# iscc/iscc-search

Hardware: AMD Instinct MI355X
Metric: queries/sec (+ roofline of the dominant kernel), 64-bit Hamming k=10 over 100M codes, exact top-k (higher is better)
Workload: dtype fp4 (e2m1 0/1 x +-1 products, f32 accumulation: exact integers)

## Files before the change

iscc_search_amd/csrc/isccsearch.hip:

```cpp
#include <hip/hip_runtime.h>

#include <algorithm>
#include <cerrno>
#include <cstdarg>
#include <cstdio>
#include <cmath>
#include <condition_variable>
#include <cstring>
#include <memory>
#include <mutex>
#include <string>
#include <unordered_map>
#include <thread>
#include <atomic>
#include <functional>
#include <chrono>
#include <vector>

#include "../../include/isccsearch.h"
#include "kernels.hip.h"
#include "mfma_scan.h"
#include "docfreq.h"
#include "simprint_score.h"
#include "asset_score.h"
// ... 110 lines not shown
        hipError_t e = hipHostMalloc((void**)&p, want * sizeof(T), hipHostMallocDefault);
        if (e != hipSuccess) { p = nullptr; (void)hipGetLastError(); return fail(-ENOMEM, "hipHostMalloc(%zu bytes) failed: %s", want * sizeof(T), hipGetErrorString(e)); }
        n = want;
        return 0;
    }
    void release() { if (p) (void)hipHostFree(p); p = nullptr; n = 0; }
};

constexpr size_t DIRECT_RESULT_BYTES = 1 << 20;

uint64_t mask_for(uint32_t pbytes) {
    const uint32_t rem = pbytes & 7;
    return rem ? ~0ULL << (8 * (8 - rem)) : ~0ULL;
}
uint32_t next_pow2(uint32_t v) { uint32_t p = 2; while (p < v) p <<= 1; return p; }

}

struct PendingSearch;
struct isccsearch_handle {
    std::mutex mu;
    std::mutex qmu;
    std::condition_variable qcv;
    std::vector<PendingSearch*> pending;
    bool leader_active = false;
    int device = 0;
    int cus = 256;
    hipStream_t stream = nullptr;
    std::vector<std::unique_ptr<Table>> tables;
    int tq = 8;
    bool profile = false;
    bool count_candidates = false;
    bool nontemporal = true;
    uint32_t blocks_per_cu = 8;
    uint64_t boot_rows = 65536;
    uint64_t level_growth = 8;
    bool repick = true;
    uint32_t tiny_rows = 16384;
    uint32_t select_wide_from = 2048;
    uint32_t fold_tau = 11;
    uint64_t stretch_bytes = CACHE_STRETCH_BYTES;
    uint64_t mfma_stretch_factor = 3;
    bool mfma = true;
    uint32_t mfma_pack_min_queries = 9;
    uint64_t mfma_few_rows = 12ull << 20;
    uint32_t mfma_min_queries = 17;
    uint32_t self_boot_per_k = 1024;
    bool spec_suppress = false;
    int device_search_hint = -1;
    int self_hint = 1;
    int speculate = 1;
    uint32_t spec_max_queries = 128;
    int mfma_pack = 1;
    uint64_t mfma_min_rows = 65536;
    bool self_tighten = true;
    bool boot_multi = true;
    uint32_t candidate_cap = 16384;
    uint32_t self_refresh_steps = 1;
    uint32_t self_max_k = ISCCSEARCH_MAX_K;
    uint64_t self_boot_rows = 65536;
    uint64_t mfma_level_growth = 4;
    uint16_t* d_rank = nullptr;
    DevBuf<uint64_t> d_queries;
    DevBuf<uint32_t> d_bias, d_cnt, d_ghist, d_overflow, d_listcnt, d_outcnt, d_freq;
    DevBuf<float> d_thr;
    DevBuf<uint64_t> d_cand;
    DevBuf<isk::Record> d_lists, d_final;
    PinBuf<uint64_t> p_queries;
    PinBuf<uint32_t> p_flags;
    DevBuf<unsigned char> d_block;
    PinBuf<unsigned char> p_block;
    DevBuf<uint64_t> d_misc;
    DevBuf<uint64_t> d_misc2;
    std::vector<isk::Record> h_final;
    std::vector<uint32_t> h_cnt, h_overflow;
    DevBuf<isk::Record> d_sp_rec;
    DevBuf<uint32_t> d_sp_rows, d_sp_nbest, d_sp_offs, d_sp_freqq, d_sp_unknown, d_sp_entry[2], d_sp_order[2], d_sp_matches, d_sp_nassets;
    DevBuf<uint32_t> d_sp_cnt, d_sp_dofg;
    DevBuf<unsigned char> d_sp_best, d_sp_temp;
    DevBuf<uint64_t> d_sp_asset[2];
    DevBuf<double> d_sp_score[2], d_sp_tab, d_sp_ws, d_sp_idfq;
    PinBuf<double> p_sp_tab;
    PinBuf<unsigned char> p_sp_out;
    uint32_t sp_tab_bits = 0, sp_tab_dup = 0xFFFFFFFFu;
    int64_t sp_tab_total = -1;
    DevBuf<isk::Record> d_am_rec, d_am_rec2;
    DevBuf<uint32_t> d_am_cnt, d_am_cnt2, d_am_off;
    DevBuf<iskas::Slot> d_am_slots;
    DevBuf<uint64_t> d_am_ex;
    DevBuf<uint8_t> d_am_hasex;
    DevBuf<double> d_am_tab;
    std::vector<double> am_tab;
    DevBuf<iskas::Item> d_am_scratch;
    PinBuf<unsigned char> p_am_out;
    size_t am_lds_allowed = 0;
    hipEvent_t ev_done = nullptr, ev_staged = nullptr, ev_producer = nullptr;
    bool ev_staged_pending = false;
    std::vector<std::pair<hipEvent_t, hipEvent_t>> ev_pool;
    std::vector<char> ev_level;
    size_t ev_used = 0;
    isccsearch_stats stats{};
};

namespace {

using H = isccsearch_handle;
// ... 232 lines not shown
        const Job& j = jobs[ji];
        Segment& s = *j.seg;
        Ctx c{};
        for (uint32_t w = 0; w < j.W; ++w) c.sp.col[w] = s.col[w];
        c.sp.queries = h->d_queries.p; c.sp.bias = h->d_bias.p; c.sp.cnt = h->d_cnt.p; c.sp.cand = h->d_cand.p;
        c.sp.ghist = h->d_ghist.p; c.sp.cap = cap; c.sp.k = k; c.sp.fold_tau = h->fold_tau; c.sp.nq_pad = nq_pad;
        c.sp.mask_lo = (uint32_t)j.mask_last; c.sp.mask_hi = (uint32_t)(j.mask_last >> 32);
        c.sp.thr_live = h->d_thr.p;
        c.sp.refresh_steps = h->self_refresh_steps;
        c.sl.cnt = h->d_cnt.p; c.sl.cand = h->d_cand.p; c.sl.cap = cap; c.sl.keys = s.keys;
        c.sl.rank = h->d_rank + (t.metric == ISCCSEARCH_METRIC_NPHD ? j.pbytes * 257 : 0);
        c.sl.out = multi ? h->d_lists.p + ji * (size_t)nq * k : d_out;
        c.sl.out_count = multi ? h->d_listcnt.p + ji * (size_t)nq : d_out_cnt;
        c.sl.overflow = d_flags + ji * (size_t)nq_pad;
        c.sl.k = k; c.sl.P = P; c.sl.prefix_bits = j.pbytes * 8; c.sl.q_base = 0;
        c.sl.overflow_count = mark_overflow ? isk::COUNT_OVERFLOW : 0;
        c.sl.out_rows = multi ? nullptr : d_out_rows;
        c.sl.out_kth = multi ? nullptr : d_out_kth;
        return c;
    }
    template <int NT>
    void launch_select_nt(const isk::SelectParams& sl, uint32_t blocks) const {
        if (sl.out_rows) {
            if (t.key_words == 2) hipLaunchKernelGGL((isk::select_kernel<2, true, NT>), dim3(blocks), dim3(NT), sel_lds, h->stream, sl);
            else hipLaunchKernelGGL((isk::select_kernel<1, true, NT>), dim3(blocks), dim3(NT), sel_lds, h->stream, sl);
        } else if (t.key_words == 2) hipLaunchKernelGGL((isk::select_kernel<2, false, NT>), dim3(blocks), dim3(NT), sel_lds, h->stream, sl);
        else hipLaunchKernelGGL((isk::select_kernel<1, false, NT>), dim3(blocks), dim3(NT), sel_lds, h->stream, sl);
    }
    void launch_select(const isk::SelectParams& sl, uint32_t blocks) const {
        const bool wide = sl.P >= h->select_wide_from && (sl.P >= 2 * h->select_wide_from || blocks <= (uint32_t)h->cus / 2);
        if (wide) launch_select_nt<1024>(sl, blocks);
        else launch_select_nt<isk::BLOCK>(sl, blocks);
    }
    bool tiny(const Job& j) const { return h->tiny_rows && j.seg->n <= h->tiny_rows && j.seg->n <= cap && j.seg->n < h->mfma_min_rows; }
    template <int NT>
    void launch_tiny_nt(const isk::TinyParams& tp, const isk::SelectParams& sl, const isk::InlineQueries& iq) const {
        if (sl.out_rows) {
            if (t.key_words == 2) hipLaunchKernelGGL((isk::tiny_search_kernel<2, true, NT>), dim3(nq), dim3(NT), sel_lds, h->stream, tp, sl, iq);
            else hipLaunchKernelGGL((isk::tiny_search_kernel<1, true, NT>), dim3(nq), dim3(NT), sel_lds, h->stream, tp, sl, iq);
        } else if (t.key_words == 2) hipLaunchKernelGGL((isk::tiny_search_kernel<2, false, NT>), dim3(nq), dim3(NT), sel_lds, h->stream, tp, sl, iq);
        else hipLaunchKernelGGL((isk::tiny_search_kernel<1, false, NT>), dim3(nq), dim3(NT), sel_lds, h->stream, tp, sl, iq);
    }
    size_t flag_words() const { return jobs.size() * (size_t)nq_pad; }

    bool use_mfma(const Job& j, uint64_t rows) const {
        const bool from_nine = j.pack || j.seg->n <= h->mfma_few_rows;
        return h->mfma && nq_pad >= (from_nine ? std::min(h->mfma_min_queries, h->mfma_pack_min_queries) : h->mfma_min_queries) && rows >= h->mfma_min_rows;
    }
    int scan(const Job& j, const isk::ScanParams& sp, int mode, bool sample) {
        const uint64_t rows = sp.n_rows - sp.row_begin;
        if (use_mfma(j, rows) || mode == isk::MODE_SELF) {
            const uint32_t g = isk::mfma_groups_per_chunk((int)j.W, nq_pad, j.pack);
            const uint32_t chunks = (nq_pad + g * 32 - 1) / (g * 32);
            const uint64_t rps = isk::mfma_rows_per_wave_step((int)j.W, j.pack);
            const uint64_t steps = (rows + rps - 1) / rps;
            const uint64_t wpb = isk::mfma_waves_per_block();
            const uint64_t bx = std::max<uint64_t>(1, std::min<uint64_t>((steps + wpb - 1) / wpb, std::max<uint32_t>(1, (uint32_t)h->cus * isk::mfma_blocks_per_cu((int)j.W, g, j.pack) / chunks)));
            const int e = isk::launch_mfma_scan((int)j.W, mode, j.pack, (uint32_t)bx, g, h->stream, sp);
            if (e) return fail(-EIO, "mfma scan: chunk of %u query groups does not fit the LDS budget (%s)", g, hipGetErrorString((hipError_t)e));
            h->stats.mfma_launches += 1;
            if (j.pack) h->stats.mfma_pack_launches += 1;
            h->stats.mfma_pair_words += rows * (uint64_t)nq * j.W;
            return 0;
        }
        if (mode != isk::MODE_COLLECT && mode != isk::MODE_STRETCH && mode != isk::MODE_BOTH) return fail(-EINVAL, "scan mode %d has no XOR + popcount kernel", mode);
        if (sp.n_rows / (uint64_t)tile_rows_for((int)j.W) >= (1ull << 31)) return fail(-E2BIG, "segment of %llu rows exceeds the scan kernel's 2^31 tiles", (unsigned long long)sp.n_rows);
        launch_scan((int)j.W, j.mask, tq, mode, h->nontemporal, dim3(scan_grid_x(h, j.W, rows, groups, sample), groups), h->stream, sp);
        return 0;
    }

    int begin(const uint64_t* hq) {
        jobs.clear();
        used_self = false;
        tq = h->tq;
        if (tq == 8 && nq > 8 && nq <= 16) tq = 16;
        nq_pad = (nq + tq - 1) / tq * tq;
        groups = nq_pad / tq;
        for (uint32_t b = 1; b <= ISCCSEARCH_MAX_BYTES; ++b) {
            Segment& s = t.seg[b];
            if (!s.n) continue;
            Job j;
            j.seg = &s;
            j.pbytes = t.metric == ISCCSEARCH_METRIC_NPHD ? std::min(b, qbytes) : b;
            j.W = (j.pbytes + 7) / 8;
            j.mask = (j.pbytes & 7) != 0;
            j.mask_last = mask_for(j.pbytes);
            j.pack = h->mfma_pack && j.W == 1;
            if (j.pack && j.pbytes == 8)
                for (uint32_t q = 0; q < nq && j.pack; ++q) j.pack = hq[(size_t)q * t.max_words] != 0;
            jobs.push_back(j);
        }
        if (jobs.empty()) {
            HIPOK(hipMemsetAsync(d_out_cnt, 0, nq * sizeof(uint32_t), h->stream));
            return 0;
        }
        cap = std::max<uint32_t>(h->candidate_cap, 16 * k);
        if (h->self_tighten && h->mfma && k <= h->self_max_k && radius < 0 && radius_ratio < 0) cap = std::max<uint32_t>(cap, 64 * k);
        multi = jobs.size() > 1;
        P = next_pow2(std::max<uint32_t>(std::max<uint32_t>(k, 1024), std::min<uint32_t>(4 * k, 4096)));
        sel_lds = (((size_t)P * 4 + 15) & ~(size_t)15) + (size_t)P * 8 * t.key_words + (d_out_rows ? (size_t)P * 4 : 0);
        int rc;
        if ((rc = h->d_queries.ensure((size_t)nq_pad * 4))) return rc;
        if ((rc = h->d_bias.ensure(nq_pad))) return rc;
        if ((rc = h->d_thr.ensure(nq_pad))) return rc;
        if ((rc = h->d_cnt.ensure((size_t)nq_pad * isk::CNT_STRIDE))) return rc;
        if ((rc = h->d_ghist.ensure((size_t)nq_pad * isk::HB))) return rc;
        if (!d_flags) {
            if ((rc = h->d_overflow.ensure(flag_words()))) return rc;
            d_flags = h->d_overflow.p;
        }
        if ((rc = h->d_cand.ensure((size_t)nq_pad * cap))) return rc;
// ... 489 lines not shown
        h->d_sp_tab.release(); h->p_sp_tab.release(); h->p_sp_out.release(); h->d_sp_ws.release(); h->d_sp_idfq.release();
        h->d_am_rec.release(); h->d_am_rec2.release(); h->d_am_cnt.release(); h->d_am_cnt2.release(); h->d_am_off.release();
        h->d_am_slots.release(); h->d_am_ex.release(); h->d_am_hasex.release(); h->d_am_tab.release(); h->d_am_scratch.release();
        h->p_am_out.release();
        if (h->d_rank) (void)hipFree(h->d_rank);
        for (auto& ev : h->ev_pool) { (void)hipEventDestroy(ev.first); (void)hipEventDestroy(ev.second); }
        for (hipEvent_t e : {h->ev_done, h->ev_staged, h->ev_producer}) if (e) (void)hipEventDestroy(e);
        if (h->stream) (void)hipStreamDestroy(h->stream);
    }
    delete h;
    return 0;
}

int isccsearch_set_option(isccsearch_handle* h, const char* name, int64_t value) {
    if (!h || !name) return fail(-EINVAL, "bad arguments");
    std::lock_guard<std::mutex> lk(h->mu);
    if (!strcmp(name, "queries_per_pass")) {
        if (value != 8 && value != 16) return fail(-EINVAL, "queries_per_pass must be 8 or 16");
        h->tq = (int)value;
        h->stats.queries_per_pass = (uint32_t)value;
        return 0;
    }
    if (!strcmp(name, "profile")) { h->profile = value != 0; return 0; }
    if (!strcmp(name, "count_candidates")) { h->count_candidates = value != 0; return 0; }
    if (!strcmp(name, "nontemporal")) {
        if (value == 0) return fail(-EINVAL, "nontemporal=0 is not available: the scan kernels are built with non-temporal loads only");
        return 0;
    }
    if (!strcmp(name, "fold")) { h->fold_tau = value ? 11 : 0; return 0; }
    if (!strcmp(name, "blocks_per_cu")) { if (value < 1 || value > 64) return fail(-EINVAL, "blocks_per_cu must be 1..64"); h->blocks_per_cu = (uint32_t)value; return 0; }
    if (!strcmp(name, "boot_rows")) { if (value < 256 || value > 65536) return fail(-EINVAL, "boot_rows must be 256..65536"); h->boot_rows = (uint64_t)value; return 0; }
    if (!strcmp(name, "mfma_stretch_factor")) { if (value < 1 || value > 64) return fail(-EINVAL, "mfma_stretch_factor must be 1..64"); h->mfma_stretch_factor = (uint64_t)value; return 0; }
    if (!strcmp(name, "stretch_mb")) { if (value < 0 || value > 65536) return fail(-EINVAL, "stretch_mb must be 0..65536"); h->stretch_bytes = (uint64_t)value << 20; return 0; }
    if (!strcmp(name, "repick")) { h->repick = value != 0; return 0; }
    if (!strcmp(name, "fold_tau")) { if (value < 0 || value > 32) return fail(-EINVAL, "fold_tau must be 0..32"); h->fold_tau = (uint32_t)value; return 0; }
    if (!strcmp(name, "level_growth")) { if (value < 2 || value > 1024) return fail(-EINVAL, "level_growth must be 2..1024"); h->level_growth = (uint64_t)value; return 0; }
    if (!strcmp(name, "mfma")) { h->mfma = value != 0; return 0; }
    if (!strcmp(name, "device_search_hint")) { if (value < -1 || value > 8 * ISCCSEARCH_MAX_BYTES) return fail(-EINVAL, "device_search_hint must be -1..256"); h->device_search_hint = (int)value; return 0; }
    if (!strcmp(name, "self_hint")) { h->self_hint = value != 0; return 0; }
    if (!strcmp(name, "mfma_few_rows")) { if (value < 0) return fail(-EINVAL, "mfma_few_rows must be >= 0"); h->mfma_few_rows = (uint64_t)value; return 0; }
    if (!strcmp(name, "mfma_pack_min_queries")) { if (value < 1 || value > 1024) return fail(-EINVAL, "mfma_pack_min_queries must be 1..1024"); h->mfma_pack_min_queries = (uint32_t)value; return 0; }
    if (!strcmp(name, "mfma_min_queries")) { if (value < 1 || value > 1024) return fail(-EINVAL, "mfma_min_queries must be 1..1024"); h->mfma_min_queries = (uint32_t)value; return 0; }
    if (!strcmp(name, "self_tighten")) { h->self_tighten = value != 0; return 0; }
    if (!strcmp(name, "boot_multi")) { h->boot_multi = value != 0; return 0; }
    if (!strcmp(name, "self_refresh_steps")) {
        if (value < 1 || value > 64 || (value & (value - 1))) return fail(-EINVAL, "self_refresh_steps must be a power of two in 1..64");
        h->self_refresh_steps = (uint32_t)value; return 0;
    }
    if (!strcmp(name, "candidate_cap")) { if (value < 64 || value > (1 << 22)) return fail(-EINVAL, "candidate_cap must be 64..4194304"); h->candidate_cap = (uint32_t)value; return 0; }
    if (!strcmp(name, "self_max_k")) { if (value < 1 || value > ISCCSEARCH_MAX_K) return fail(-EINVAL, "self_max_k must be 1..%d", ISCCSEARCH_MAX_K); h->self_max_k = (uint32_t)value; return 0; }
    if (!strcmp(name, "self_boot_rows")) { if (value < 256 || value > (1 << 20)) return fail(-EINVAL, "self_boot_rows must be 256..1048576"); h->self_boot_rows = (uint64_t)value; return 0; }
    if (!strcmp(name, "mfma_level_growth")) { if (value < 2 || value > 1024) return fail(-EINVAL, "mfma_level_growth must be 2..1024"); h->mfma_level_growth = (uint64_t)value; return 0; }
    if (!strcmp(name, "mfma_pack")) { h->mfma_pack = value != 0; return 0; }
    if (!strcmp(name, "tiny_rows")) { if (value < 0 || value > (1 << 20)) return fail(-EINVAL, "tiny_rows must be 0..1048576"); h->tiny_rows = (uint32_t)value; return 0; }
    if (!strcmp(name, "select_wide_from")) { if (value < 0) return fail(-EINVAL, "select_wide_from must be >= 0"); h->select_wide_from = (uint32_t)std::min<int64_t>(value, 0xFFFFFFFFll); return 0; }
    if (!strcmp(name, "speculate")) { h->speculate = value != 0; return 0; }
    if (!strcmp(name, "spec_max_queries")) { if (value < 0 || value > 1024) return fail(-EINVAL, "spec_max_queries must be 0..1024"); h->spec_max_queries = (uint32_t)value; return 0; }
    if (!strcmp(name, "self_boot_per_k")) { if (value < 0 || value > (1 << 20)) return fail(-EINVAL, "self_boot_per_k must be 0..2^20"); h->self_boot_per_k = (uint32_t)value; return 0; }
    if (!strcmp(name, "mfma_min_rows")) { if (value < 1) return fail(-EINVAL, "mfma_min_rows must be >= 1"); h->mfma_min_rows = (uint64_t)value; return 0; }
    if (!strcmp(name, "sample_cost")) return 0;
    return fail(-EINVAL, "unknown option '%s'", name);
}

int isccsearch_stats_get(isccsearch_handle* h, isccsearch_stats* out, int reset) {
    if (!h || !out) return fail(-EINVAL, "bad arguments");
    std::lock_guard<std::mutex> lk(h->mu);
    HIPOK(hipSetDevice(h->device));
    int rc = drain_events(h);
    if (rc) return rc;
    *out = h->stats;
    if (reset) {
        const uint32_t tq = h->stats.queries_per_pass, cu = h->stats.compute_units;
        h->stats = isccsearch_stats{};
        h->stats.queries_per_pass = tq;
        h->stats.compute_units = cu;
    }
    return 0;
}

int isccsearch_table_open(isccsearch_handle* h, int metric, int key_words, int max_bytes, uint32_t* table_id) {
    if (!h || !table_id) return fail(-EINVAL, "bad arguments");
    if (metric != ISCCSEARCH_METRIC_HAMMING && metric != ISCCSEARCH_METRIC_NPHD) return fail(-EINVAL, "unknown metric %d", metric);
    if (key_words != 1 && key_words != 2) return fail(-EINVAL, "key_words must be 1 or 2");
    if (max_bytes < 1 || max_bytes > ISCCSEARCH_MAX_BYTES) return fail(-EINVAL, "max_bytes must be 1..%d", ISCCSEARCH_MAX_BYTES);
    std::lock_guard<std::mutex> lk(h->mu);
    std::unique_ptr<Table> t(new Table());
    t->open = true;
    t->metric = metric;
    t->key_words = key_words;
    t->max_bytes = max_bytes;
    t->max_words = (max_bytes + 7) / 8;
    for (uint32_t b = 1; b <= ISCCSEARCH_MAX_BYTES; ++b) { t->seg[b].nbytes = b; t->seg[b].W = (b + 7) / 8; }
    for (size_t i = 0; i < h->tables.size(); ++i)
        if (!h->tables[i]) { h->tables[i] = std::move(t); *table_id = (uint32_t)i; return 0; }
    h->tables.push_back(std::move(t));
    *table_id = (uint32_t)(h->tables.size() - 1);
    return 0;
}

int isccsearch_table_drop(isccsearch_handle* h, uint32_t table) {
    if (!h) return fail(-EINVAL, "handle is NULL");
    std::lock_guard<std::mutex> lk(h->mu);
    Table* t;
    int rc = get_table(h, table, t);
    if (rc) return rc;
    HIPOK(hipSetDevice(h->device));
// ... 1646 lines not shown
```

iscc_search_amd/csrc/mfma_scan.h:

```cpp
#pragma once

#include <hip/hip_runtime.h>
#include <stddef.h>
#include <stdint.h>

#include "scan_params.hip.h"

namespace isk {

constexpr int MFMA_MAX_LDS = 48 * 1024;

uint32_t mfma_groups_per_chunk(int W, uint32_t nq_pad, bool pack);
size_t mfma_lds_bytes(int W, uint32_t groups);
uint32_t mfma_waves_per_block();
uint32_t mfma_rows_per_wave_step(int W, bool pack);
uint32_t mfma_blocks_per_cu(int W, uint32_t groups, bool pack);
int launch_mfma_scan(int W, int mode, bool pack, uint32_t blocks_x, uint32_t groups, hipStream_t st, const ScanParams& p);

}
```

iscc_search_amd/csrc/mfma_scan.hip:

```cpp
#include "mfma_scan.h"

#include <hip/hip_runtime.h>

namespace isk {

typedef int v4i __attribute__((ext_vector_type(4)));
typedef uint32_t u32x4 __attribute__((ext_vector_type(4)));
typedef int v8i __attribute__((ext_vector_type(8)));
typedef float v16f __attribute__((ext_vector_type(16)));
typedef const __attribute__((address_space(3))) v4i* lds_frag_ptr;
typedef const __attribute__((address_space(3))) float* lds_thr_ptr;

#ifndef ISK_MFMA_TILES_W4
#define ISK_MFMA_TILES_W4 2
#endif
template <int W> constexpr int mfma_tiles() { return W == 4 ? ISK_MFMA_TILES_W4 : 2; }
#ifndef ISK_ORDERED_STAGE
#define ISK_ORDERED_STAGE 0
#endif
#ifndef ISK_EXP_NO_CANDIDATE_MEMORY
#define ISK_EXP_NO_CANDIDATE_MEMORY 0
#endif
#ifndef ISK_SCALAR_STEPS_FROM_W
#define ISK_SCALAR_STEPS_FROM_W 2
#endif
constexpr uint32_t PK_RING_ENTRIES = 8, PK_RING_ENTRY_DWORDS = 36;
constexpr int MBLOCK = 256;
template <int W> constexpr int mfma_min_waves() { return W <= 3 ? 3 : (mfma_tiles<W>() == 1 ? 4 : 2); }
constexpr int FP4 = 4;
constexpr int SCALE_ONE = 0;

__device__ __forceinline__ float min3f(float a, float b, float c) { return fminf(fminf(a, b), c); }
__device__ __forceinline__ float live_threshold(const float* addr) {
    return __int_as_float(__hip_atomic_load(reinterpret_cast<const int*>(addr), __ATOMIC_RELAXED, __HIP_MEMORY_SCOPE_AGENT));
}

__device__ __forceinline__ uint32_t nibbles(uint32_t x, int j) { return (x >> j) & 0x11111111u; }

template <int N>
__device__ __forceinline__ void fold_op(float& mA, float& mB, const v16f& o0, const v16f& o1) {
    if constexpr (N == 0) asm volatile("v_min3_f32 %0, %1, %2, %3" : "=v"(mA) : "v"(o0[0]), "v"(o0[1]), "v"(o0[2]));
    else if constexpr (N <= 6) asm volatile("v_min3_f32 %0, %0, %1, %2" : "+v"(mA) : "v"(o0[2 * N + 1]), "v"(o0[2 * N + 2]));
    else if constexpr (N == 7) asm volatile("v_min3_f32 %0, %1, %2, %3" : "=v"(mB) : "v"(o1[0]), "v"(o1[1]), "v"(o1[2]));
    else if constexpr (N <= 13) asm volatile("v_min3_f32 %0, %0, %1, %2" : "+v"(mB) : "v"(o1[2 * (N - 7) + 1]), "v"(o1[2 * (N - 7) + 2]));
    else if constexpr (N == 14) asm volatile("v_min3_f32 %0, %0, %1, %2" : "+v"(mA) : "v"(o0[15]), "v"(o1[15]));
    else asm volatile("v_min_f32 %0, %0, %1" : "+v"(mA) : "v"(mB));
}
template <int FROM, int TO>
__device__ __forceinline__ void fold_ops(float& mA, float& mB, const v16f& o0, const v16f& o1) {
    if constexpr (FROM < TO && FROM < 16) {
        fold_op<FROM>(mA, mB, o0, o1);
        fold_ops<FROM + 1, TO>(mA, mB, o0, o1);
    }
}
template <bool FIRST_WORD>
__device__ __forceinline__ void mfma_asm(v16f& acc, const v4i& a, const v4i& b) {
    if constexpr (FIRST_WORD) asm volatile("v_mfma_f32_32x32x64_f8f6f4 %0, %1, %2, 0 cbsz:4 blgp:4" : "=&v"(acc) : "v"(a), "v"(b));
    else asm volatile("v_mfma_f32_32x32x64_f8f6f4 %0, %1, %2, %0 cbsz:4 blgp:4" : "+v"(acc) : "v"(a), "v"(b));
}

// ... 756 lines not shown
                ++trip;
            }
            even_flush(step - stride);
        }
    } else {
        const uint64_t nfull = p.n_rows / (32 * MT);
        const uint64_t leap = stride * STRETCH;
        constexpr int HOP = STRETCH == 1 ? 0 : 1;
        u32x4 x[DEPTH];
#pragma unroll
        for (int d = 0; d < DEPTH; ++d) x[d] = u32x4{0u, 0u, 0u, 0u};
        if (step < nfull) {
            uint64_t base = step, last = step;
            uint32_t last_d = 0;
            bool more = true;
#pragma unroll
            for (int d = 0; d < DEPTH; ++d) issue_rows(x[d], base + (HOP ? d : d * stride) < nfull ? base + (HOP ? d : d * stride) : base);
            while (more) {
#pragma unroll
                for (int d = 0; d < DEPTH; ++d) {
                    step = base + (HOP ? d : d * stride);
                    if (step >= nfull) { more = false; break; }
                    const uint64_t prev = HOP ? (d ? step - 1 : step - leap + (DEPTH - 1)) : step - stride;
                    const uint64_t ahead = HOP ? leap : stride * DEPTH;
                    await_rows(x[d]);
                    expand(x[d]);
                    issue_rows(x[d], step + ahead < nfull ? step + ahead : base);
                    if constexpr (G == 0) one_step(all_groups);
                    else if constexpr ((G & 1) != 0) {
                        static_assert((DEPTH & 1) == 0, "the accumulator roles of an odd group count alternate with d");
                        if (d & 1) one_step([&]() __attribute__((always_inline)) { few_step(accY, accX, prev); });
                        else one_step([&]() __attribute__((always_inline)) { few_step(accX, accY, prev); });
                        last_d = d;
                    } else one_step([&]() __attribute__((always_inline)) { few_step(accX, accY, prev); });
                    last = step;
                    ++trip;
                }
                if (more) { base += HOP ? leap : stride * DEPTH; step = base; }
            }
            asm volatile("s_waitcnt vmcnt(0)" ::: "memory");
            if constexpr ((G & 1) != 0) {
                if (last_d & 1) few_flush(accY, last);
                else few_flush(accX, last);
            } else if constexpr (G > 1) few_flush(accY, last);
        }
        if (step < nsteps) {
            expand(load_rows(step));
            one_step(all_groups);
        }
    }
    if constexpr (MODE == MODE_SELF) pend_complete();
}

template <int DEPTH, int G>
static void launch_pack_depth(int mode, dim3 grid, size_t lds, hipStream_t st, const ScanParams& p, uint32_t groups) {
    if (mode == MODE_COLLECT) hipLaunchKernelGGL((mfma_pack_kernel<MODE_COLLECT, DEPTH, G>), grid, dim3(MBLOCK), lds, st, p, groups);
    else if (mode == MODE_STRETCH) hipLaunchKernelGGL((mfma_pack_kernel<MODE_STRETCH, DEPTH, G>), grid, dim3(MBLOCK), lds, st, p, groups);
    else if (mode == MODE_SELF) hipLaunchKernelGGL((mfma_pack_kernel<MODE_SELF, DEPTH, G>), grid, dim3(MBLOCK), lds, st, p, groups);
    else hipLaunchKernelGGL((mfma_pack_kernel<MODE_BOTH, DEPTH, G>), grid, dim3(MBLOCK), lds, st, p, groups);
}

static int launch_pack(int mode, dim3 grid, size_t lds, hipStream_t st, const ScanParams& p, uint32_t groups) {
    if (lds > (size_t)MFMA_MAX_LDS) return (int)hipErrorInvalidValue;
    static_assert(PK_DEEP_GROUPS == 4, "one case per count");
    switch (groups) {
        case 1: launch_pack_depth<4, 1>(mode, grid, lds, st, p, groups); break;
        case 2: launch_pack_depth<4, 2>(mode, grid, lds, st, p, groups); break;
        case 3: launch_pack_depth<4, 3>(mode, grid, lds, st, p, groups); break;
        case 4: launch_pack_depth<4, 4>(mode, grid, lds, st, p, groups); break;
        default: launch_pack_depth<1, 0>(mode, grid, lds, st, p, groups);
    }
    return 0;
}

template <int W>
static int launch_w(int mode, dim3 grid, size_t lds, hipStream_t st, const ScanParams& p, uint32_t groups) {
    if (lds > (size_t)MFMA_MAX_LDS) return (int)hipErrorInvalidValue;
    if (mode == MODE_COLLECT) hipLaunchKernelGGL((mfma_scan_kernel<W, MODE_COLLECT>), grid, dim3(MBLOCK), lds, st, p, groups);
    else if (mode == MODE_STRETCH) hipLaunchKernelGGL((mfma_scan_kernel<W, MODE_STRETCH>), grid, dim3(MBLOCK), lds, st, p, groups);
    else if (mode == MODE_SELF) hipLaunchKernelGGL((mfma_scan_kernel<W, MODE_SELF>), grid, dim3(MBLOCK), lds, st, p, groups);
    else hipLaunchKernelGGL((mfma_scan_kernel<W, MODE_BOTH>), grid, dim3(MBLOCK), lds, st, p, groups);
    return 0;
}

uint32_t mfma_groups_per_chunk(int W, uint32_t nq_pad, bool pack) {
    static const uint32_t max_groups[5] = {0, 32, 16, 10, 8};
    uint32_t need = (nq_pad + 31) / 32;
    if (pack) return need < 1 ? 1 : (need < max_groups[1] ? need : max_groups[1]);
    need += need & 1;
    if (need < 2) need = 2;
    if (need <= max_groups[W]) return need;
    const uint32_t chunks = (need + max_groups[W] - 1) / max_groups[W];
    uint32_t g = (need + chunks - 1) / chunks;
    g += g & 1;
    return g < max_groups[W] ? g : max_groups[W];
}

size_t mfma_lds_bytes(int W, uint32_t groups) { return (size_t)groups * W * 64 * 16 + (size_t)groups * 32 * 8 + MBLOCK / 64 * PK_RING_ENTRIES * PK_RING_ENTRY_DWORDS * sizeof(uint32_t); }

uint32_t mfma_waves_per_block() { return MBLOCK / 64; }
uint32_t mfma_rows_per_wave_step(int W, bool pack) { return pack ? 32u * PK_TILES : 32u * (uint32_t)(W == 4 ? mfma_tiles<4>() : 2); }

uint32_t mfma_blocks_per_cu(int W, uint32_t groups, bool pack) {
    const uint32_t by_lds = (uint32_t)((160u * 1024u) / mfma_lds_bytes(W, groups));
    const uint32_t by_regs = pack || W <= 3 ? 3u : (mfma_tiles<4>() == 1 ? 4u : 2u);
    return by_lds < by_regs ? (by_lds ? by_lds : 1u) : by_regs;
}

int launch_mfma_scan(int W, int mode, bool pack, uint32_t blocks_x, uint32_t groups, hipStream_t st, const ScanParams& p) {
    const uint32_t chunks = (p.nq_pad + groups * 32 - 1) / (groups * 32);
    const dim3 grid(blocks_x, chunks);
    const size_t lds = mfma_lds_bytes(W, groups);
    if (pack) return W == 1 ? launch_pack(mode, grid, lds, st, p, groups) : (int)hipErrorInvalidValue;
    switch (W) {
        case 1: return launch_w<1>(mode, grid, lds, st, p, groups);
        case 2: return launch_w<2>(mode, grid, lds, st, p, groups);
        case 3: return launch_w<3>(mode, grid, lds, st, p, groups);
        default: return launch_w<4>(mode, grid, lds, st, p, groups);
    }
}

}
```

Before: 446,900.

## Add packed MFMA scan kernel that folds three Hamming distances per accumulator

Adds a new pack3 MFMA kernel for 64-bit codes with more than four query groups. It encodes query and row bits as fp4 so that scaled f8f6f4 MFMAs (scale factors 2^7 and 2^14) pack three distance sums into one f32 lane. Threshold tests are then done with OR3/bitop3 masks instead of per-distance compares. It is meant to cut the number of MFMA output registers and the compare work per row, at the cost of complex bit-field decoding, a threshold-biased start value, and a larger 192-row step per wave. The path is enabled by default and can be switched off with a new knob.

```diff
diff --git a/iscc_search_amd/csrc/isccsearch.hip b/iscc_search_amd/csrc/isccsearch.hip
--- a/iscc_search_amd/csrc/isccsearch.hip
+++ b/iscc_search_amd/csrc/isccsearch.hip
@@ -186,6 +186,7 @@
     int speculate = 1;
     uint32_t spec_max_queries = 128;
     int mfma_pack = 1;
+    int mfma_pack3 = 1;
     uint64_t mfma_min_rows = 65536;
     bool self_tighten = true;
     bool boot_multi = true;
@@ -524,11 +525,12 @@
         if (use_mfma(j, rows) || mode == isk::MODE_SELF) {
             const uint32_t g = isk::mfma_groups_per_chunk((int)j.W, nq_pad, j.pack);
             const uint32_t chunks = (nq_pad + g * 32 - 1) / (g * 32);
-            const uint64_t rps = isk::mfma_rows_per_wave_step((int)j.W, j.pack);
+            const bool pack3 = j.pack && h->mfma_pack3 && isk::mfma_pack3_fits(g);
+            const uint64_t rps = isk::mfma_rows_per_wave_step((int)j.W, j.pack, pack3);
             const uint64_t steps = (rows + rps - 1) / rps;
             const uint64_t wpb = isk::mfma_waves_per_block();
             const uint64_t bx = std::max<uint64_t>(1, std::min<uint64_t>((steps + wpb - 1) / wpb, std::max<uint32_t>(1, (uint32_t)h->cus * isk::mfma_blocks_per_cu((int)j.W, g, j.pack) / chunks)));
-            const int e = isk::launch_mfma_scan((int)j.W, mode, j.pack, (uint32_t)bx, g, h->stream, sp);
+            const int e = isk::launch_mfma_scan((int)j.W, mode, j.pack, (uint32_t)bx, g, h->stream, sp, pack3);
             if (e) return fail(-EIO, "mfma scan: chunk of %u query groups does not fit the LDS budget (%s)", g, hipGetErrorString((hipError_t)e));
             h->stats.mfma_launches += 1;
             if (j.pack) h->stats.mfma_pack_launches += 1;
@@ -1124,6 +1126,7 @@
     if (!strcmp(name, "self_boot_rows")) { if (value < 256 || value > (1 << 20)) return fail(-EINVAL, "self_boot_rows must be 256..1048576"); h->self_boot_rows = (uint64_t)value; return 0; }
     if (!strcmp(name, "mfma_level_growth")) { if (value < 2 || value > 1024) return fail(-EINVAL, "mfma_level_growth must be 2..1024"); h->mfma_level_growth = (uint64_t)value; return 0; }
     if (!strcmp(name, "mfma_pack")) { h->mfma_pack = value != 0; return 0; }
+    if (!strcmp(name, "mfma_pack3")) { h->mfma_pack3 = value != 0; return 0; }
     if (!strcmp(name, "tiny_rows")) { if (value < 0 || value > (1 << 20)) return fail(-EINVAL, "tiny_rows must be 0..1048576"); h->tiny_rows = (uint32_t)value; return 0; }
     if (!strcmp(name, "select_wide_from")) { if (value < 0) return fail(-EINVAL, "select_wide_from must be >= 0"); h->select_wide_from = (uint32_t)std::min<int64_t>(value, 0xFFFFFFFFll); return 0; }
     if (!strcmp(name, "speculate")) { h->speculate = value != 0; return 0; }
diff --git a/iscc_search_amd/csrc/mfma_scan.h b/iscc_search_amd/csrc/mfma_scan.h
--- a/iscc_search_amd/csrc/mfma_scan.h
+++ b/iscc_search_amd/csrc/mfma_scan.h
@@ -13,8 +13,9 @@
 uint32_t mfma_groups_per_chunk(int W, uint32_t nq_pad, bool pack);
 size_t mfma_lds_bytes(int W, uint32_t groups);
 uint32_t mfma_waves_per_block();
-uint32_t mfma_rows_per_wave_step(int W, bool pack);
+bool mfma_pack3_fits(uint32_t groups);
+uint32_t mfma_rows_per_wave_step(int W, bool pack, bool pack3 = false);
 uint32_t mfma_blocks_per_cu(int W, uint32_t groups, bool pack);
-int launch_mfma_scan(int W, int mode, bool pack, uint32_t blocks_x, uint32_t groups, hipStream_t st, const ScanParams& p);
+int launch_mfma_scan(int W, int mode, bool pack, uint32_t blocks_x, uint32_t groups, hipStream_t st, const ScanParams& p, bool pack3 = false);
 
 }
diff --git a/iscc_search_amd/csrc/mfma_scan.hip b/iscc_search_amd/csrc/mfma_scan.hip
--- a/iscc_search_amd/csrc/mfma_scan.hip
+++ b/iscc_search_amd/csrc/mfma_scan.hip
@@ -6,6 +6,7 @@
 
 typedef int v4i __attribute__((ext_vector_type(4)));
 typedef uint32_t u32x4 __attribute__((ext_vector_type(4)));
+typedef uint32_t u32x2 __attribute__((ext_vector_type(2)));
 typedef int v8i __attribute__((ext_vector_type(8)));
 typedef float v16f __attribute__((ext_vector_type(16)));
 typedef const __attribute__((address_space(3))) v4i* lds_frag_ptr;
@@ -868,6 +869,408 @@
     if constexpr (MODE == MODE_SELF) pend_complete();
 }
 
+constexpr int P3_TILES = 6;
+constexpr uint32_t P3_IND = 0x00204080u;
+constexpr uint32_t P3_LDS_EXTRA = 16;
+
+__host__ __device__ __forceinline__ uint32_t p3_start(uint32_t T, uint32_t m) {
+    const uint32_t bias = 63 + T - m / 2;
+    return 0x4B000000u | (bias << 1) | (bias << 8) | (bias << 15);
+}
+__device__ __forceinline__ v4i p3_rows(uint32_t x) {
+    return v4i{(int)((x & 0x88888888u) | 0x22222222u), (int)(((x << 1) & 0x88888888u) | 0x22222222u),
+               (int)(((x << 2) & 0x88888888u) | 0x22222222u), (int)(((x << 3) & 0x88888888u) | 0x22222222u)};
+}
+__device__ __forceinline__ int p3_tau1(uint32_t tpk, int pc) {
+    const int t = unpack_threshold(tpk) + pc;
+    return (t < -1 ? -1 : t > 64 ? 64 : t) + 1;
+}
+__device__ __forceinline__ int p3_wave_max(int v) {
+    v = max(v, __builtin_amdgcn_update_dpp(0, v, 0x111, 0xF, 0xF, false));
+    v = max(v, __builtin_amdgcn_update_dpp(0, v, 0x112, 0xF, 0xF, false));
+    v = max(v, __builtin_amdgcn_update_dpp(0, v, 0x114, 0xF, 0xF, false));
+    v = max(v, __builtin_amdgcn_update_dpp(0, v, 0x118, 0xF, 0xF, false));
+    v = max(v, __builtin_amdgcn_update_dpp(0, v, 0x142, 0xF, 0xF, false));
+    v = max(v, __builtin_amdgcn_update_dpp(0, v, 0x143, 0xF, 0xF, false));
+    return __builtin_amdgcn_readlane(v, 63);
+}
+
+#define ISK_P3A(n, av) "v_mfma_f32_32x32x64_f8f6f4 %[" #n "], %[" #av "], %[b], %[st] cbsz:4 blgp:4\n"
+#define ISK_P3B(n, av) "v_mfma_scale_f32_32x32x64_f8f6f4 %[" #n "], %[" #av "], %[b], %[" #n "], %[s7], %[so] op_sel_hi:[0,0,0] cbsz:4 blgp:4\n"
+#define ISK_P3C(n, av) "v_mfma_scale_f32_32x32x64_f8f6f4 %[" #n "], %[" #av "], %[b], %[" #n "], %[s14], %[so] op_sel_hi:[0,0,0] cbsz:4 blgp:4\n"
+#define ISK_OR3(d, x, y, z) "v_or3_b32 %[" #d "], %[" #x "], %[" #y "], %[" #z "]\n"
+
+template <int MODE, bool ODD>
+__global__ __launch_bounds__(MBLOCK, 3) void mfma_pack3_kernel(const ScanParams p, const uint32_t groups) {
+    constexpr uint32_t ROWS = 32 * P3_TILES;
+    constexpr uint32_t RING_E = PK_RING_ENTRIES, ENTRY = PK_RING_ENTRY_DWORDS;
+    extern __shared__ __attribute__((aligned(16))) unsigned char smem[];
+    v4i* lb = reinterpret_cast<v4i*>(smem);
+    uint32_t* lthr = reinterpret_cast<uint32_t*>(smem + (size_t)groups * 64 * 16);
+    int* lpop = reinterpret_cast<int*>(lthr + groups * 32);
+    uint32_t* const rings = reinterpret_cast<uint32_t*>(lpop + groups * 32);
+    int* const lmax = reinterpret_cast<int*>(rings + (MBLOCK / 64) * RING_E * ENTRY);
+    const uint32_t tid = threadIdx.x, lane = tid & 63, wave = tid >> 6;
+    const uint32_t q0 = blockIdx.y * groups * 32;
+    const uint32_t mbits = (uint32_t)(__popc(p.mask_lo) + __popc(p.mask_hi));
+
+    for (uint32_t i = tid; i < groups * 32 * 2; i += MBLOCK) {
+        const uint32_t ql = i >> 1, hh = i & 1;
+        const uint32_t q = q0 + ql;
+        const bool live = q < p.nq_pad && p.bias[q] != BIAS_NEVER;
+        const uint64_t qw = live ? p.queries[(uint64_t)q * 4] : 0;
+        const uint32_t x = hh ? (uint32_t)(qw >> 32) : (uint32_t)qw;
+        const uint32_t m = live ? (hh ? p.mask_hi : p.mask_lo) : 0u;
+        const uint32_t g = ql >> 5, c = ql & 31;
+        v4i frag;
+#pragma unroll
+        for (int j = 0; j < 4; ++j) frag[j] = (int)((((x << j) & 0x88888888u) | 0x22222222u) & ((((m << j) & 0x88888888u) >> 3) * 0xFu));
+        lb[(size_t)g * 64 + hh * 32 + c] = frag;
+    }
+    for (uint32_t ql = tid; ql < groups * 32; ql += MBLOCK) {
+        const uint32_t q = q0 + ql;
+        int pc = 0, tau = -1;
+        if (q < p.nq_pad) {
+            pc = __popcll(p.queries[(uint64_t)q * 4] & (((uint64_t)p.mask_hi << 32) | p.mask_lo));
+            tau = (int)(0x7FFFFFFFu - p.bias[q]);
+        }
+        lpop[ql] = pc;
+        if constexpr (MODE == MODE_SELF) lthr[ql] = q < p.nq_pad ? live_packed(p.thr_live + q) : 0u;
+        else lthr[ql] = pack_threshold(tau - pc);
+    }
+    __syncthreads();
+
+    const uint32_t wave_s = (uint32_t)__builtin_amdgcn_readfirstlane((int)wave);
+    auto fresh_index = [&]() __attribute__((always_inline)) {
+        uint32_t z = 0;
+        asm volatile("" : "+v"(z));
+        return wave_s * 256 + __builtin_amdgcn_mbcnt_hi(~0u, __builtin_amdgcn_mbcnt_lo(~0u, z)) * 4;
+    };
+    const bool mine4 = wave * 256 + lane * 4 < groups * 32;
+    auto publish_max = [&](const uint32_t (&t4)[4], bool valid) __attribute__((always_inline)) {
+        int v = 0;
+        if (valid) {
+            const int4 pc = *reinterpret_cast<const int4*>(lpop + fresh_index());
+            v = max(max(p3_tau1(t4[0], pc.x), p3_tau1(t4[1], pc.y)), max(p3_tau1(t4[2], pc.z), p3_tau1(t4[3], pc.w)));
+        }
+        v = p3_wave_max(v);
+        if (lane == 0) lmax[wave] = v;
+    };
+    {
+        uint32_t t4[4] = {0u, 0u, 0u, 0u};
+        if (mine4) {
+            const uint4 v = *reinterpret_cast<const uint4*>(lthr + fresh_index());
+            t4[0] = v.x; t4[1] = v.y; t4[2] = v.z; t4[3] = v.w;
+        }
+        publish_max(t4, mine4);
+    }
+    __syncthreads();
+
+    const uint64_t nsteps = (p.n_rows - p.row_begin + ROWS - 1) / ROWS;
+    const uint64_t stride = (uint64_t)gridDim.x * (MBLOCK / 64);
+    uint64_t step = (uint64_t)blockIdx.x * (MBLOCK / 64) + wave_s;
+    if (step >= nsteps) return;
+    const uint64_t last_row = p.n_rows - 1;
+    const uint32_t* const col32 = reinterpret_cast<const uint32_t*>(p.col[0]);
+
+    uint32_t tcur = 65;
+    const float s0 = __uint_as_float(p3_start(64, mbits));
+    v16f start = {s0, s0, s0, s0, s0, s0, s0, s0, s0, s0, s0, s0, s0, s0, s0, s0};
+    auto update_t = [&]() __attribute__((always_inline)) {
+        const int4 mx = *reinterpret_cast<const int4*>(lmax);
+        const uint32_t t1 = (uint32_t)__builtin_amdgcn_readfirstlane(max(max(mx.x, mx.y), max(mx.z, mx.w)));
+        const uint32_t tn = t1 < 1 ? 1u : t1;
+        if (tn < tcur) {
+            tcur = tn;
+            const float sv = __uint_as_float(p3_start(tn > 64 ? 64u : tn, mbits));
+            start = v16f{sv, sv, sv, sv, sv, sv, sv, sv, sv, sv, sv, sv, sv, sv, sv, sv};
+        }
+        asm volatile("" : "+v"(start));
+    };
+    update_t();
+    auto t_of = [](uint32_t t) { return t > 64 ? 64u : t; };
+    auto ind_of = [](uint32_t t) { return t > 64 ? P3_IND | 0x40000000u : P3_IND; };
+
+    struct Acc { v16f t[2]; };
+    uint32_t rcount = 0;
+    uint32_t pend_slot = 0, pend_lo = 0, pend_hi = 0x80000000u;
+    auto pend_complete = [&]() __attribute__((always_inline)) {
+        if (!(pend_hi & 0x80000000u)) {
+            const uint32_t qi = q0 + (pend_hi >> 20);
+            if (pend_slot < p.cap) p.cand[(uint64_t)qi * p.cap + pend_slot] = ((uint64_t)((pend_hi >> 12) & 0x7Fu) << 48) | ((uint64_t)(pend_hi & 0xFFFu) << 32) | pend_lo;
+            pend_hi = 0x80000000u;
+        }
+    };
+    auto lane_now = [&]() __attribute__((always_inline)) {
+        uint32_t z = 0;
+        asm volatile("" : "+v"(z));
+        return __builtin_amdgcn_mbcnt_hi(~0u, __builtin_amdgcn_mbcnt_lo(~0u, z));
+    };
+    auto process_ring = [&](uint64_t st) __attribute__((always_inline)) {
+        const uint32_t ln = lane_now(), sub = ln >> 5, reg = ln & 31, i = reg & 15, acc = reg >> 4;
+        const uint32_t m0 = (i & 3) + 8 * (i >> 2);
+        const uint64_t row0 = p.row_begin + st * ROWS;
+        for (uint32_t e = 0; e < rcount; e += 2) {
+            if (e + sub < rcount) {
+                const uint32_t* const blk = rings + wave_s * (RING_E * ENTRY) + (e + sub) * ENTRY;
+                const uint32_t bits = blk[reg], head = blk[32], tb = blk[33];
+                const uint32_t ql = head & 0xFFFFu, mm = m0 + 4 * (head >> 16);
+                const int pc = lpop[ql];
+                const int tau = unpack_threshold(lthr[ql]) + pc;
+#pragma unroll 1
+                for (int f = 0; f < 3; ++f) {
+                    const int d = 63 + (int)tb - (int)((bits >> (1 + 7 * f)) & 0x7Fu);
+                    const uint32_t t = 3 * acc + f;
+                    const uint64_t row = row0 + (t < 4 ? 2 * mm + 64 * (t & 1) + (t >> 1) : 128 + 32 * (t - 4) + mm);
+                    if (d <= tau && d >= 0 && row <= last_row) {
+                        if constexpr (MODE == MODE_SELF) {
+                            pend_complete();
+                            const uint32_t qi = q0 + ql, hd = (uint32_t)d;
+                            pend_slot = atomicAdd(&p.cnt[(uint64_t)qi * CNT_STRIDE], 1u);
+                            uint32_t* const counts = p.ghist + (uint64_t)qi * HB;
+                            for (int tt = d; tt < tau; ++tt) __hip_atomic_fetch_add(&counts[tt], 1u, __ATOMIC_RELAXED, __HIP_MEMORY_SCOPE_AGENT);
+                            pend_lo = (uint32_t)row;
+                            pend_hi = (ql << 20) | (hd << 12) | (uint32_t)(row >> 32);
+                        } else {
+                            emit<MODE>(p, q0 + ql, (uint32_t)d, row);
+                        }
+                    }
+                }
+            }
+        }
+        rcount = 0;
+    };
+    auto save_hits = [&](const Acc& a2, uint64_t mask, uint32_t tb, uint32_t g, uint64_t st) __attribute__((always_inline)) {
+        while (mask) {
+            const uint32_t room = RING_E - rcount;
+            if (room == 0) { process_ring(st); continue; }
+            const uint32_t rank = __builtin_amdgcn_mbcnt_hi((uint32_t)(mask >> 32), __builtin_amdgcn_mbcnt_lo((uint32_t)mask, 0u));
+            const uint32_t ln = lane_now();
+            const bool mine = ((mask >> ln) & 1) != 0 && rank < room;
+            if (mine) {
+                uint32_t* const blk = rings + wave_s * (RING_E * ENTRY) + (rcount + rank) * ENTRY;
+#pragma unroll
+                for (int j = 0; j < 2; ++j)
+#pragma unroll
+                    for (int i = 0; i < 16; i += 4)
+                        *reinterpret_cast<float4*>(blk + 16 * j + i) = make_float4(a2.t[j][i], a2.t[j][i + 1], a2.t[j][i + 2], a2.t[j][i + 3]);
+                *reinterpret_cast<uint2*>(blk + 32) = make_uint2((g * 32 + (ln & 31)) | ((ln >> 5) << 16), tb);
+            }
+            const uint64_t taken = __builtin_amdgcn_ballot_w64(mine);
+            rcount += (uint32_t)__builtin_popcountll(taken);
+            mask &= ~taken;
+        }
+    };
+
+    int sc7 = (int)0x86868686, sc14 = (int)0x8D8D8D8D, sc_one = 0x7F7F7F7F;
+    asm volatile("" : "+v"(sc7), "+v"(sc14), "+v"(sc_one));
+    v4i a[P3_TILES];
+
+    auto stage = [&](Acc& nw, const Acc& od, const v4i& b, uint32_t ind) __attribute__((always_inline)) -> uint64_t {
+        uint32_t oA, oB, rr;
+        uint64_t mask;
+        const v16f& u = od.t[0];
+        const v16f& w = od.t[1];
+        asm volatile(ISK_P3A(n0, a0)
+                     ISK_OR3(A, u0, u1, u2) ISK_OR3(B, u3, u4, u5) ISK_OR3(A, A, u6, u7)
+                     : [n0] "=&v"(nw.t[0]), [A] "=&v"(oA), [B] "=&v"(oB)
+                     : [a0] "v"(a[0]), [b] "v"(b), [st] "v"(start), [u0] "v"(u[0]), [u1] "v"(u[1]), [u2] "v"(u[2]), [u3] "v"(u[3]), [u4] "v"(u[4]),
+                       [u5] "v"(u[5]), [u6] "v"(u[6]), [u7] "v"(u[7]));
+        asm volatile(ISK_P3B(n0, a1)
+                     ISK_OR3(B, B, u8, u9) ISK_OR3(A, A, u10, u11) ISK_OR3(B, B, u12, u13)
+                     : [n0] "+v"(nw.t[0]), [A] "+v"(oA), [B] "+v"(oB)
+                     : [a1] "v"(a[1]), [b] "v"(b), [s7] "v"(sc7), [so] "v"(sc_one), [u8] "v"(u[8]), [u9] "v"(u[9]), [u10] "v"(u[10]), [u11] "v"(u[11]),
+                       [u12] "v"(u[12]), [u13] "v"(u[13]));
+        asm volatile(ISK_P3C(n0, a2)
+                     ISK_OR3(A, A, u14, u15) ISK_OR3(B, B, w0, w1) ISK_OR3(A, A, w2, w3)
+                     : [n0] "+v"(nw.t[0]), [A] "+v"(oA), [B] "+v"(oB)
+                     : [a2] "v"(a[2]), [b] "v"(b), [s14] "v"(sc14), [so] "v"(sc_one), [u14] "v"(u[14]), [u15] "v"(u[15]), [w0] "v"(w[0]), [w1] "v"(w[1]),
+                       [w2] "v"(w[2]), [w3] "v"(w[3]));
+        asm volatile(ISK_P3A(n1, a3)
+                     ISK_OR3(B, B, w4, w5) ISK_OR3(A, A, w6, w7) ISK_OR3(B, B, w8, w9)
+                     : [n1] "=&v"(nw.t[1]), [A] "+v"(oA), [B] "+v"(oB)
+                     : [a3] "v"(a[3]), [b] "v"(b), [st] "v"(start), [w4] "v"(w[4]), [w5] "v"(w[5]), [w6] "v"(w[6]), [w7] "v"(w[7]),
+                       [w8] "v"(w[8]), [w9] "v"(w[9]));
+        asm volatile(ISK_P3B(n1, a4)
+                     ISK_OR3(A, A, w10, w11) ISK_OR3(B, B, w12, w13) ISK_OR3(A, A, w14, w15)
+                     : [n1] "+v"(nw.t[1]), [A] "+v"(oA), [B] "+v"(oB)
+                     : [a4] "v"(a[4]), [b] "v"(b), [s7] "v"(sc7), [so] "v"(sc_one), [w10] "v"(w[10]), [w11] "v"(w[11]), [w12] "v"(w[12]), [w13] "v"(w[13]),
+                       [w14] "v"(w[14]), [w15] "v"(w[15]));
+        asm volatile(ISK_P3C(n1, a5)
+                     "v_bitop3_b32 %[R], %[A], %[B], %[ind] bitop3:0xa8\n"
+                     "v_cmp_ne_u32_e64 %[mask], %[R], 0\n"
+                     : [n1] "+v"(nw.t[1]), [R] "=&v"(rr), [mask] "=s"(mask)
+                     : [a5] "v"(a[5]), [b] "v"(b), [s14] "v"(sc14), [so] "v"(sc_one), [A] "v"(oA), [B] "v"(oB), [ind] "s"(ind));
+        return mask;
+    };
+    auto first_group = [&](Acc& nw, const v4i& b) __attribute__((always_inline)) {
+        asm volatile(ISK_P3A(n0, a0) ISK_P3B(n0, a1) ISK_P3C(n0, a2) ISK_P3A(n1, a3) ISK_P3B(n1, a4) ISK_P3C(n1, a5) "s_nop 7\ns_nop 3\n"
+                     : [n0] "=&v"(nw.t[0]), [n1] "=&v"(nw.t[1])
+                     : [a0] "v"(a[0]), [a1] "v"(a[1]), [a2] "v"(a[2]), [a3] "v"(a[3]), [a4] "v"(a[4]), [a5] "v"(a[5]), [b] "v"(b), [st] "v"(start),
+                       [s7] "v"(sc7), [s14] "v"(sc14), [so] "v"(sc_one));
+    };
+    auto last_fold = [&](const Acc& od, uint32_t ind) __attribute__((always_inline)) -> uint64_t {
+        uint32_t oA, oB, rr;
+        uint64_t mask;
+        const v16f& u = od.t[0];
+        const v16f& w = od.t[1];
+        asm volatile("s_nop 7\ns_nop 3\n"
+                     ISK_OR3(A, u0, u1, u2) ISK_OR3(B, u3, u4, u5) ISK_OR3(A, A, u6, u7) ISK_OR3(B, B, u8, u9)
+                     ISK_OR3(A, A, u10, u11) ISK_OR3(B, B, u12, u13) ISK_OR3(A, A, u14, u15)
+                     : [A] "=&v"(oA), [B] "=&v"(oB)
+                     : [u0] "v"(u[0]), [u1] "v"(u[1]), [u2] "v"(u[2]), [u3] "v"(u[3]), [u4] "v"(u[4]), [u5] "v"(u[5]), [u6] "v"(u[6]), [u7] "v"(u[7]),
+                       [u8] "v"(u[8]), [u9] "v"(u[9]), [u10] "v"(u[10]), [u11] "v"(u[11]), [u12] "v"(u[12]), [u13] "v"(u[13]), [u14] "v"(u[14]), [u15] "v"(u[15]));
+        asm volatile(ISK_OR3(B, B, w0, w1) ISK_OR3(A, A, w2, w3) ISK_OR3(B, B, w4, w5) ISK_OR3(A, A, w6, w7)
+                     ISK_OR3(B, B, w8, w9) ISK_OR3(A, A, w10, w11) ISK_OR3(B, B, w12, w13) ISK_OR3(A, A, w14, w15)
+                     "v_bitop3_b32 %[R], %[A], %[B], %[ind] bitop3:0xa8\n"
+                     "v_cmp_ne_u32_e64 %[mask], %[R], 0\n"
+                     : [A] "+v"(oA), [B] "+v"(oB), [R] "=&v"(rr), [mask] "=s"(mask)
+                     : [w0] "v"(w[0]), [w1] "v"(w[1]), [w2] "v"(w[2]), [w3] "v"(w[3]), [w4] "v"(w[4]), [w5] "v"(w[5]), [w6] "v"(w[6]), [w7] "v"(w[7]),
+                       [w8] "v"(w[8]), [w9] "v"(w[9]), [w10] "v"(w[10]), [w11] "v"(w[11]), [w12] "v"(w[12]), [w13] "v"(w[13]), [w14] "v"(w[14]), [w15] "v"(w[15]),
+                       [ind] "s"(ind));
+        return mask;
+    };
+
+    const v4i* const lbl = lb + lane;
+    struct Rows { u32x4 x; u32x2 y; };
+    auto load_rows = [&](uint64_t st) __attribute__((always_inline)) -> Rows {
+        const uint64_t row0 = p.row_begin + st * ROWS;
+        if (row0 + ROWS <= p.n_rows)
+            return Rows{__builtin_nontemporal_load(reinterpret_cast<const u32x4*>(col32 + row0 * 2) + lane),
+                        __builtin_nontemporal_load(reinterpret_cast<const u32x2*>(col32 + (row0 + 128) * 2) + lane)};
+        const uint64_t r0 = row0 + 2 * lane, r1 = r0 + 1, r2 = row0 + 128 + lane;
+        const uint2 lo = *reinterpret_cast<const uint2*>(col32 + (r0 <= last_row ? r0 : last_row) * 2);
+        const uint2 hi = *reinterpret_cast<const uint2*>(col32 + (r1 <= last_row ? r1 : last_row) * 2);
+        const uint2 th = *reinterpret_cast<const uint2*>(col32 + (r2 <= last_row ? r2 : last_row) * 2);
+        return Rows{u32x4{lo.x, lo.y, hi.x, hi.y}, u32x2{th.x, th.y}};
+    };
+    auto expand = [&](const Rows& v) __attribute__((always_inline)) {
+        const auto e = __builtin_amdgcn_permlane32_swap(v.x[0], v.x[1], false, false);
+        const auto o = __builtin_amdgcn_permlane32_swap(v.x[2], v.x[3], false, false);
+        const auto f = __builtin_amdgcn_permlane32_swap(v.y[0], v.y[1], false, false);
+        a[0] = p3_rows(e[0]);
+        a[1] = p3_rows(e[1]);
+        a[2] = p3_rows(o[0]);
+        a[3] = p3_rows(o[1]);
+        a[4] = p3_rows(f[0]);
+        a[5] = p3_rows(f[1]);
+    };
+
+    const bool refresh = MODE == MODE_SELF && mine4 && q0 + wave * 256 + lane * 4 < p.nq_pad;
+    const uint32_t refresh_mask = (groups >= 32 ? 1u : groups >= 16 ? 2u : groups >= 8 ? 4u : 8u) * ((p.refresh_steps + 1) / 2) - 1u;
+    const uint32_t slices = groups * 32 * 4 / 64, nwaves = gridDim.x * (MBLOCK / 64);
+    const uint32_t gw = blockIdx.x * (MBLOCK / 64) + wave_s;
+    uint32_t trip = 0;
+    Acc accX, accY;
+    auto all_groups = [&]() __attribute__((always_inline)) {
+        v4i by = lbl[0], bx = lbl[64];
+        const uint32_t tb = t_of(tcur), ind = ind_of(tcur);
+        first_group(accY, by);
+        uint32_t g = 0;
+#pragma unroll 1
+        for (; g + 2 < groups; g += 2) {
+            by = lbl[(g + 2) * 64];
+            if (const uint64_t mk = stage(accX, accY, bx, ind); __builtin_expect(mk != 0, 0)) save_hits(accY, mk, tb, g, step);
+            const uint32_t g3 = g + 3 < groups ? g + 3 : g + 2;
+            bx = lbl[g3 * 64];
+            if (const uint64_t mk = stage(accY, accX, by, ind); __builtin_expect(mk != 0, 0)) save_hits(accX, mk, tb, g + 1, step);
+        }
+        if (g + 1 < groups) {
+            if (const uint64_t mk = stage(accX, accY, bx, ind); mk != 0) save_hits(accY, mk, tb, g, step);
+            if (const uint64_t mk = last_fold(accX, ind); mk != 0) save_hits(accX, mk, tb, g + 1, step);
+        } else {
+            if (const uint64_t mk = last_fold(accY, ind); mk != 0) save_hits(accY, mk, tb, g, step);
+        }
+    };
+    bool carried = false;
+    uint32_t tcar = 64;
+    auto even_groups = [&](uint64_t prev) __attribute__((always_inline)) {
+        v4i by = lbl[0], bx = lbl[64];
+        const uint32_t tb = t_of(tcur), ind = ind_of(tcur);
+        if (const uint64_t mk = stage(accY, accX, by, ind_of(tcar)); __builtin_expect(carried && mk != 0, 0)) { save_hits(accX, mk, t_of(tcar), groups - 1, prev); process_ring(prev); }
+        uint32_t g = 0;
+#pragma unroll 1
+        for (; g + 2 < groups; g += 2) {
+            by = lbl[(g + 2) * 64];
+            if (const uint64_t mk = stage(accX, accY, bx, ind); __builtin_expect(mk != 0, 0)) save_hits(accY, mk, tb, g, step);
+            bx = lbl[(g + 3) * 64];
+            if (const uint64_t mk = stage(accY, accX, by, ind); __builtin_expect(mk != 0, 0)) save_hits(accX, mk, tb, g + 1, step);
+        }
+        if (const uint64_t mk = stage(accX, accY, bx, ind); __builtin_expect(mk != 0, 0)) save_hits(accY, mk, tb, g, step);
+        carried = true;
+        tcar = tcur;
+    };
+    auto even_flush = [&](uint64_t prev) __attribute__((always_inline)) {
+        if (carried) {
+            if (const uint64_t mk = last_fold(accX, ind_of(tcar)); mk != 0) { save_hits(accX, mk, t_of(tcar), groups - 1, prev); process_ring(prev); }
+            carried = false;
+        }
+    };
+    auto one_step = [&](auto&& body) __attribute__((always_inline)) {
+        uint32_t fresh[4] = {0u, 0u, 0u, 0u};
+        const bool look = trip < 4 || (trip & refresh_mask) == 0;
+        const bool refresh_now = refresh && look;
+        if constexpr (MODE == MODE_SELF) {
+            if (look) update_t();
+        }
+        body();
+        if constexpr (MODE == MODE_SELF) pend_complete();
+        if (rcount) process_ring(step);
+        if constexpr (MODE == MODE_SELF) {
+            uint32_t chk_count = 0, chk_what = ~0u;
+            const uint32_t slice = nwaves >= slices ? gw : (gw + trip * nwaves) % slices;
+            if (look && slice < slices) {
+                uint32_t z = 0;
+                asm volatile("" : "+v"(z));
+                const uint32_t task = slice * 64 + __builtin_amdgcn_mbcnt_hi(~0u, __builtin_amdgcn_mbcnt_lo(~0u, z));
+                const uint32_t ql = task >> 2, tpk = lthr[ql];
+                const int level = unpack_threshold(tpk) + lpop[ql] - 1 - (int)(task & 3);
+                if (tpk != 0 && level >= 0 && q0 + ql < p.nq_pad) {
+                    chk_what = ql | ((uint32_t)level << 16);
+                    chk_count = (uint32_t)__hip_atomic_load(reinterpret_cast<const int*>(p.ghist + (uint64_t)(q0 + ql) * HB + level), __ATOMIC_RELAXED, __HIP_MEMORY_SCOPE_AGENT);
+                }
+            }
+            if (refresh_now) {
+                const float* const src = p.thr_live + q0 + fresh_index();
+#pragma unroll
+                for (int i = 0; i < 4; ++i) fresh[i] = live_packed(src + i);
+            }
+            if (chk_what != ~0u && chk_count >= p.k) {
+                const uint32_t ql = chk_what & 0xFFFFu;
+                atomicMin(reinterpret_cast<uint32_t*>(p.thr_live) + q0 + ql, pack_threshold((int)(chk_what >> 16) - lpop[ql]));
+            }
+            if (refresh_now) *reinterpret_cast<uint4*>(lthr + fresh_index()) = make_uint4(fresh[0], fresh[1], fresh[2], fresh[3]);
+            if (look) publish_max(fresh, refresh_now);
+        }
+    };
+    Rows x = load_rows(step);
+    if constexpr (ODD) {
+        while (step < nsteps) {
+            expand(x);
+            x = load_rows(step + stride < nsteps ? step + stride : step);
+            one_step(all_groups);
+            step += stride;
+            ++trip;
+        }
+    } else {
+        while (step < nsteps) {
+            expand(x);
+            x = load_rows(step + stride < nsteps ? step + stride : step);
+            one_step([&]() __attribute__((always_inline)) { even_groups(step - stride); });
+            step += stride;
+            ++trip;
+        }
+        even_flush(step - stride);
+    }
+    if constexpr (MODE == MODE_SELF) pend_complete();
+}
+
+template <int MODE>
+static void launch_pack3_mode(dim3 grid, size_t lds, hipStream_t st, const ScanParams& p, uint32_t groups) {
+    if (groups & 1) hipLaunchKernelGGL((mfma_pack3_kernel<MODE, true>), grid, dim3(MBLOCK), lds, st, p, groups);
+    else hipLaunchKernelGGL((mfma_pack3_kernel<MODE, false>), grid, dim3(MBLOCK), lds, st, p, groups);
+}
+
 template <int DEPTH, int G>
 static void launch_pack_depth(int mode, dim3 grid, size_t lds, hipStream_t st, const ScanParams& p, uint32_t groups) {
     if (mode == MODE_COLLECT) hipLaunchKernelGGL((mfma_pack_kernel<MODE_COLLECT, DEPTH, G>), grid, dim3(MBLOCK), lds, st, p, groups);
@@ -876,7 +1279,16 @@
     else hipLaunchKernelGGL((mfma_pack_kernel<MODE_BOTH, DEPTH, G>), grid, dim3(MBLOCK), lds, st, p, groups);
 }
 
-static int launch_pack(int mode, dim3 grid, size_t lds, hipStream_t st, const ScanParams& p, uint32_t groups) {
+static int launch_pack(int mode, dim3 grid, size_t lds, hipStream_t st, const ScanParams& p, uint32_t groups, bool pack3) {
+    if (pack3 && mfma_pack3_fits(groups)) {
+        lds += P3_LDS_EXTRA;
+        if (lds > (size_t)MFMA_MAX_LDS) return (int)hipErrorInvalidValue;
+        if (mode == MODE_COLLECT) launch_pack3_mode<MODE_COLLECT>(grid, lds, st, p, groups);
+        else if (mode == MODE_STRETCH) launch_pack3_mode<MODE_STRETCH>(grid, lds, st, p, groups);
+        else if (mode == MODE_SELF) launch_pack3_mode<MODE_SELF>(grid, lds, st, p, groups);
+        else launch_pack3_mode<MODE_BOTH>(grid, lds, st, p, groups);
+        return 0;
+    }
     if (lds > (size_t)MFMA_MAX_LDS) return (int)hipErrorInvalidValue;
     static_assert(PK_DEEP_GROUPS == 4, "one case per count");
     switch (groups) {
@@ -915,7 +1327,8 @@
 size_t mfma_lds_bytes(int W, uint32_t groups) { return (size_t)groups * W * 64 * 16 + (size_t)groups * 32 * 8 + MBLOCK / 64 * PK_RING_ENTRIES * PK_RING_ENTRY_DWORDS * sizeof(uint32_t); }
 
 uint32_t mfma_waves_per_block() { return MBLOCK / 64; }
-uint32_t mfma_rows_per_wave_step(int W, bool pack) { return pack ? 32u * PK_TILES : 32u * (uint32_t)(W == 4 ? mfma_tiles<4>() : 2); }
+uint32_t mfma_rows_per_wave_step(int W, bool pack, bool pack3) { return pack3 ? 32u * P3_TILES : pack ? 32u * PK_TILES : 32u * (uint32_t)(W == 4 ? mfma_tiles<4>() : 2); }
+bool mfma_pack3_fits(uint32_t groups) { return groups > PK_DEEP_GROUPS; }
 
 uint32_t mfma_blocks_per_cu(int W, uint32_t groups, bool pack) {
     const uint32_t by_lds = (uint32_t)((160u * 1024u) / mfma_lds_bytes(W, groups));
@@ -923,11 +1336,11 @@
     return by_lds < by_regs ? (by_lds ? by_lds : 1u) : by_regs;
 }
 
-int launch_mfma_scan(int W, int mode, bool pack, uint32_t blocks_x, uint32_t groups, hipStream_t st, const ScanParams& p) {
+int launch_mfma_scan(int W, int mode, bool pack, uint32_t blocks_x, uint32_t groups, hipStream_t st, const ScanParams& p, bool pack3) {
     const uint32_t chunks = (p.nq_pad + groups * 32 - 1) / (groups * 32);
     const dim3 grid(blocks_x, chunks);
     const size_t lds = mfma_lds_bytes(W, groups);
-    if (pack) return W == 1 ? launch_pack(mode, grid, lds, st, p, groups) : (int)hipErrorInvalidValue;
+    if (pack) return W == 1 ? launch_pack(mode, grid, lds, st, p, groups, pack3) : (int)hipErrorInvalidValue;
     switch (W) {
         case 1: return launch_w<1>(mode, grid, lds, st, p, groups);
         case 2: return launch_w<2>(mode, grid, lds, st, p, groups);
```

New measurement: 515,700, median of 6. 15.4% higher.
